# DCASE-REPO/DESED_task

Measured on AMD Instinct MI355X. Metric: 10s-clips/sec CRNN mean-teacher train @batch48, higher is better.
Workload: dtype f32 (fp32 storage and accumulation; the dense contractions of the wide layers run as split-bf16 MFMA, 3 bf16 products per fp32 product, fp32-level accuracy; everything else exact f32)

## Files before the change

### desed_task_amd/csrc/sed_glu.hip

```cpp
#include "sed_common.h"

#ifndef GLU_ABL
#define GLU_ABL 0
#endif

template <int C, int PT, int PF>
struct GluGeom {
    static constexpr int WIN = PT * PF;
    static constexpr int CP = C + 1;
    static constexpr int NT = C >= 32 ? C / 32 : 1;
};

template <int PT, int PF>
__device__ __forceinline__ bool row_pixel(int m, int o0, int NWC, int fsh, int& o, int& t, int& f) {
    constexpr int WIN = PT * PF;
    const int q = m % WIN;
    o = o0 + m / WIN;
    const int to = o >> fsh, fo = o & ((1 << fsh) - 1);
    t = to * PT + q / PF;
    f = fo * PF + q % PF;
    return o < NWC;
}

template <int C, int PT, int PF>
// ... 1711 lines not shown
                const int m = 16 * rb + 4 * g + r;
                const uint32_t e_idx = (uint32_t)(row0 + m) * (uint32_t)C + (uint32_t)n;
                const float xn = fmaf(xq[r], gn, bn);
                const float sg = (GLU_ABL & 2) ? xn : sed_fast_sigmoid(xn);
                const float lin = acc[rb][r] + biasp;
                const float gq = ((GLU_ABL & 2) || sed_keep(e_idx, seed, thr24)) ? g8[2 * rb + (r >> 1)] : 0.f;
                const float dlin = gq * sg;
                const float e = gq * lin * sg * (1.0f - sg);
                bf16_split(dlin, hh[r], ll[r]);
                dh[rm_off(m, n)] = hh[r];
                dl[rm_off(m, n)] = ll[r];
                acc[rb][r] = e;
                a_dbg += dlin;
            }
            uint2 hv, lv;
            hv.x = (unsigned)hh[0] | ((unsigned)hh[1] << 16); hv.y = (unsigned)hh[2] | ((unsigned)hh[3] << 16);
            lv.x = (unsigned)ll[0] | ((unsigned)ll[1] << 16); lv.y = (unsigned)ll[2] | ((unsigned)ll[3] << 16);
            const int off = tr_off(n, 16 * rb + 4 * g);
            *(uint2*)(dth + off) = hv;
            *(uint2*)(dtl + off) = lv;
        }
        __syncthreads();
        if (!(GLU_ABL & 1)) gemm_rows(dh, b2h, b2l, acc);
        const bool full = row0 + ROWS <= R;
#pragma unroll
        for (int rb = 0; rb < RB; ++rb) {
            float xq[4];
            xhat4(rb, xq);
#pragma unroll
            for (int r = 0; r < 4; ++r) {
                const int m = 16 * rb + 4 * g + r;
                const float dxn = acc[rb][r];
                a_dgam = fmaf(dxn, xq[r], a_dgam);
                a_dbet += dxn;
                if (!(GLU_ABL & 8) && (full || row0 + m < R)) dz[(size_t)(row0 + m) * C + n] = dxn * gn;
            }
        }
        if (tile + (int)gridDim.x < ntiles) load_tile(tile + gridDim.x);
        if (!(GLU_ABL & 1)) {
            const int rowa = 16 * w + i16;
            s16x8 ah3, al3;
#pragma unroll
            for (int st = 0; st < 2 * KS3; ++st) {
                const int ks = st >> 1, c0 = 4 * (st & 1);
                if ((st & 1) == 0) {
                    const int offa = tr_off(rowa, 32 * ks + 8 * g);
                    ah3 = *(const s16x8*)(dth + offa);
                    al3 = *(const s16x8*)(dtl + offa);
                }
                s16x8 bh3[4], bl3[4];
#pragma unroll
                for (int q = 0; q < 4; ++q) {
                    const int offb = tr_off(16 * (c0 + q) + i16, 32 * ks + 8 * g);
                    bh3[q] = *(const s16x8*)(xth + offb);
                    bl3[q] = *(const s16x8*)(xtl + offb);
                }
#pragma unroll
                for (int q = 0; q < 4; ++q) P[c0 + q] = mfma16_bf16(al3, bh3[q], P[c0 + q]);
#pragma unroll
                for (int q = 0; q < 4; ++q) P[c0 + q] = mfma16_bf16(ah3, bl3[q], P[c0 + q]);
#pragma unroll
                for (int q = 0; q < 4; ++q) P[c0 + q] = mfma16_bf16(ah3, bh3[q], P[c0 + q]);
                sed_sched_fence();
            }
        }
    }
    float* mine = part + (size_t)blockIdx.x * (C * C + 3 * C);
#pragma unroll
    for (int cb = 0; cb < NB; ++cb)
#pragma unroll
        for (int r = 0; r < 4; ++r) mine[(16 * w + 4 * g + r) * C + 16 * cb + i16] = P[cb][r];
    a_dbg += __shfl_xor(a_dbg, 16); a_dgam += __shfl_xor(a_dgam, 16); a_dbet += __shfl_xor(a_dbet, 16);
    a_dbg += __shfl_xor(a_dbg, 32); a_dgam += __shfl_xor(a_dgam, 32); a_dbet += __shfl_xor(a_dbet, 32);
    if (g == 0) {
        float* dst = mine + C * C;
        dst[n] = a_dbg; dst[C + n] = a_dgam; dst[2 * C + n] = a_dbet;
    }
}
#define GBR_THREADS 1024
#define GBR_GROUPS (GBR_THREADS / 16)
__global__ __launch_bounds__(GBR_THREADS) void glu_bwd_reduce_kernel(const float* __restrict__ part, float* __restrict__ dWg,
                                                             float* __restrict__ dbg, float* __restrict__ dgamma,
                                                             float* __restrict__ dbeta, int nblk, int C, int KS, int WMS,
                                                             const float* __restrict__ gamma, const float* __restrict__ beta, int fix) {
    __shared__ float4 red[GBR_GROUPS][16];
    __shared__ float sdb[GBR_THREADS / 64];
    const int tid = threadIdx.x, col = tid & 15, grp = tid >> 4, e = blockIdx.x * 64 + 4 * col;
    const int CC = C * C, PART = KS * CC + WMS * 3 * C;
    const bool isw = e < CC;
    const int nsl = isw ? KS : WMS, sstride = isw ? CC : 3 * C;
    const size_t off = isw ? (size_t)e : (size_t)KS * CC + (e - CC);
    float4 acc = make_float4(0.f, 0.f, 0.f, 0.f);
    if (e < CC + 3 * C) {
        const int total = nblk * nsl;
#pragma unroll 4
        for (int i = grp; i < total; i += GBR_GROUPS) {
            const int b = i / nsl, k = i - b * nsl;
            const float4 v = *(const float4*)(part + (size_t)b * PART + off + (size_t)k * sstride);
            acc.x += v.x; acc.y += v.y; acc.z += v.z; acc.w += v.w;
        }
    }
    const bool need_dbn = fix && blockIdx.x * 64 < CC;
    float sacc = 0.f;
    if (need_dbn) {
        const int nrow = (blockIdx.x * 64) / C;
#pragma unroll 2
        for (int i = tid; i < nblk * WMS; i += GBR_THREADS) {
            const int b = i / WMS, k = i - b * WMS;
            sacc += part[(size_t)b * PART + (size_t)KS * CC + k * 3 * C + nrow];
        }
    }
    float4 gq = make_float4(0.f, 0.f, 0.f, 0.f), bq = gq;
    if (fix && isw && grp == 0) {
        const int c = e % C;
        gq = make_float4(gamma[c], gamma[c + 1], gamma[c + 2], gamma[c + 3]);
        bq = make_float4(beta[c], beta[c + 1], beta[c + 2], beta[c + 3]);
    }
    red[grp][col] = acc;
    if (need_dbn) {
        sacc = wave_sum(sacc);
        if ((tid & 63) == 0) sdb[tid >> 6] = sacc;
    }
    __syncthreads();
    float dbn = 0.f;
    if (need_dbn) {
#pragma unroll
        for (int w = 0; w < GBR_THREADS / 64; ++w) dbn += sdb[w];
    }
    if (grp == 0 && e < CC + 3 * C) {
#pragma unroll 8
        for (int g = 1; g < GBR_GROUPS; ++g) { const float4 v = red[g][col]; acc.x += v.x; acc.y += v.y; acc.z += v.z; acc.w += v.w; }
        if (fix && isw) {
            acc.x = fmaf(gq.x, acc.x, bq.x * dbn); acc.y = fmaf(gq.y, acc.y, bq.y * dbn);
            acc.z = fmaf(gq.z, acc.z, bq.z * dbn); acc.w = fmaf(gq.w, acc.w, bq.w * dbn);
        }
        float* dst;
        if (isw) dst = dWg + e;
        else {
            const int j2 = e - CC, which = j2 / C;
            dst = (which == 0 ? dbg : which == 1 ? dgamma : dbeta) + (j2 - which * C);
        }
        *(float4*)dst = acc;
    }
}
template <int C, bool SPLIT>
static int launch_glu_wide_bwd(const float* y, const float* stats, const float* gamma, const float* beta, const float* Wg,
                               const float* bg, const float* gout, float* dz, float* dWg, float* dbg, float* dgamma, float* dbeta,
                               float* scratch, int B, int T, int F, uint32_t seed, uint32_t thr24, float dscale, const unsigned* seed_dev, hipStream_t s) {
    constexpr int ROWS = 32 * (8 / (C / 32)), WMS = 8 / (C / 32), KS = (C / 32) * (C / 32) >= 8 ? 1 : 8 / ((C / 32) * (C / 32));
    if (!scratch) return SED_ERR_ARG;
    constexpr int SMEM = SPLIT ? 8 * (ROWS * (C + 8) + C * (ROWS + 8)) : (2 * ROWS + (C > 64 ? C : 0)) * (C + 1) * 4;
    const int ntiles = (B * T * F + ROWS - 1) / ROWS;
    const int cap = glu_grid_cap(256);
    int grid = ntiles < cap ? ntiles : cap;
    if (grid < 1) { sed_zero4(s, dWg, C * C, dbg, C, dgamma, C, dbeta, C); return SED_OK; }
    if (SPLIT && C == 128 && sed_tuning[SED_TUNE_GLU_BWD128_SPLIT] != 1) {
        constexpr int SMEM_C = 8 * 64 * 128 * 2;
        SED_MAX_SMEM(glu128_bwd_c_kernel, SMEM_C);
        SED_LAUNCH(glu128_bwd_c_kernel, dim3(grid), dim3(512), SMEM_C, s, y, stats, gamma, beta, Wg, bg, gout, dz, scratch, B, T, F,
                   seed, thr24, dscale, seed_dev);
        SED_LAUNCH(glu_bwd_reduce_kernel, dim3((C * C + 3 * C + 63) / 64), dim3(GBR_THREADS), 0, s, scratch, dWg, dbg, dgamma, dbeta, grid, C, 1, 1,
                   gamma, beta, 1);
        return sed_check_launch();
    }
    if (SPLIT) {
        SED_MAX_SMEM((glu_wide_bwd_b_kernel<C>), SMEM);
        SED_LAUNCH((glu_wide_bwd_b_kernel<C>), dim3(grid), dim3(512), SMEM, s, y, stats, gamma, beta, Wg, bg, gout, dz, scratch, B, T, F,
                   seed, thr24, dscale, seed_dev);
    } else {
        SED_MAX_SMEM((glu_wide_bwd_kernel<C>), SMEM);
        SED_LAUNCH((glu_wide_bwd_kernel<C>), dim3(grid), dim3(512), SMEM, s, y, stats, gamma, beta, Wg, bg, gout, dz, scratch, B, T, F,
                   seed, thr24, dscale, seed_dev);
    }
    SED_LAUNCH(glu_bwd_reduce_kernel, dim3((C * C + 3 * C + 63) / 64), dim3(GBR_THREADS), 0, s, scratch, dWg, dbg, dgamma, dbeta, grid, C, KS, WMS,
               gamma, beta, SPLIT ? 1 : 0);
    return sed_check_launch();
}

SED_API long long sed_glu_bwd_scratch_floats(int B, int T, int F, int C, int PT, int PF) {
    (void)B; (void)T; (void)F;
    if (PT == 1 && PF == 2 && (C == 64 || C == 128)) {
        const int nt3 = (C / 32) * (C / 32), ks = nt3 >= 8 ? 1 : 8 / nt3, wms = 8 / (C / 32);
        return 256LL * (ks * C * C + wms * 3 * C);
    }
    if (PT == 2 && PF == 2 && (C == 16 || C == 32)) return 1024LL * (C * C + 3 * C);
    return 0;
}

SED_API int sed_glu_bwd(const float* y, const float* stats, const float* gamma, const float* beta, const float* Wg,
                           const float* bg, const float* gout, float* dz, float* dWg, float* dbg, float* dgamma, float* dbeta,
                           float* scratch, int B, int T, int F, int C, int PT, int PF, unsigned seed, unsigned thr24, float dscale,
                           const unsigned* seed_dev, int split_bf16, void* stream) {
    hipStream_t s = (hipStream_t)stream;
    if (F % PF != 0) return SED_ERR_UNSUPPORTED;
    if (PT == 1 && PF == 2) {
        if (C == 128 && split_bf16 && sed_tuning[SED_TUNE_GLU_BWD128_SPLIT] != 3)
            return launch_glu_wide_bwd<128, true>(y, stats, gamma, beta, Wg, bg, gout, dz, dWg, dbg, dgamma, dbeta, scratch, B, T, F, seed, thr24, dscale, seed_dev, s);
        if (C == 64 && split_bf16) return launch_glu_wide_bwd<64, true>(y, stats, gamma, beta, Wg, bg, gout, dz, dWg, dbg, dgamma, dbeta, scratch, B, T, F, seed, thr24, dscale, seed_dev, s);
        if (C == 128) return launch_glu_wide_bwd<128, false>(y, stats, gamma, beta, Wg, bg, gout, dz, dWg, dbg, dgamma, dbeta, scratch, B, T, F, seed, thr24, dscale, seed_dev, s);
        if (C == 64) return launch_glu_wide_bwd<64, false>(y, stats, gamma, beta, Wg, bg, gout, dz, dWg, dbg, dgamma, dbeta, scratch, B, T, F, seed, thr24, dscale, seed_dev, s);
    }
    const bool lds_free32 = C == 32 && PT == 2 && PF == 2 && F % 16 == 0 && T >= 2;
    if (T % PT != 0 && !lds_free32) {
        const int tail = T % PT, rowf4 = F * C / 4;
        const long long n4 = (long long)B * tail * rowf4;
        int grid = (int)((n4 + 255) / 256);
        if (grid > 2048) grid = 2048;
        SED_LAUNCH(glu_zero_tail_kernel, dim3(grid), dim3(256), 0, s, dz, n4, T, T - tail, tail * rowf4, (long long)T * rowf4);
    }
    if ((C == 16 && PT == 2 && PF == 2 && F % 8 == 0) || (C == 32 && PT == 2 && PF == 2 && F % 16 == 0)) {
        const int nrows = B * (T / 2);
        int grid = (nrows + 3) / 4;
        const int cap = C == 32 ? glu_grid_cap(512) : 1024;
        if (grid > cap) grid = cap;
        if (grid < 1) { sed_zero4(s, dWg, C * C, dbg, C, dgamma, C, dbeta, C); return SED_OK; }
        if (!scratch) return SED_ERR_ARG;
        if (C == 16)
            SED_LAUNCH(glu16_bwd_kernel, dim3(grid), dim3(256), 0, s, y, stats, gamma, beta, Wg, bg, gout, dz, scratch, B, T, F, seed, thr24,
                       dscale, seed_dev);
        else
            SED_LAUNCH(glu32_bwd_kernel, dim3(grid), dim3(256), 0, s, y, stats, gamma, beta, Wg, bg, gout, dz, scratch, B, T, F, seed, thr24,
                       dscale, seed_dev);
        SED_LAUNCH(glu_bwd_reduce_kernel, dim3((C * C + 3 * C + 63) / 64), dim3(GBR_THREADS), 0, s, scratch, dWg, dbg, dgamma, dbeta, grid, C, 1, 1,
                   gamma, beta, 0);
        return sed_check_launch();
    }
    sed_zero4(s, dWg, C * C, dbg, C, dgamma, C, dbeta, C);
#define GLU_CASE(c, pt, pf)                                                                                              \
    if (C == c && PT == pt && PF == pf)                                                                                  \
        return launch_glu_bwd<c, pt, pf>(y, stats, gamma, beta, Wg, bg, gout, dz, dWg, dbg, dgamma, dbeta, B, T, F, seed, thr24, \
                                         dscale, seed_dev, s);
    GLU_CASE(16, 2, 2) GLU_CASE(32, 2, 2)
#undef GLU_CASE
    return SED_ERR_UNSUPPORTED;
}

template <int C>
__global__ __launch_bounds__(256) void bn_bwd_apply_kernel(const float* __restrict__ y, float* __restrict__ dz,
                                                           const float* __restrict__ stats, const float* __restrict__ gamma,
                                                           const float* __restrict__ dgamma, const float* __restrict__ dbeta,
                                                           float* __restrict__ dbias, size_t npix, float inv_count, int training) {
    constexpr int V = C / 4, RPI = 256 / V;
    const int tid = threadIdx.x, v = tid % V, r0 = tid / V;
    float mean[4], istd[4], m1[4], m2[4];
#pragma unroll
    for (int i = 0; i < 4; ++i) {
        const int c = 4 * v + i;
        mean[i] = stats[c];
        istd[i] = stats[C + c];
        m1[i] = training ? gamma[c] * dbeta[c] * inv_count : 0.f;
        m2[i] = training ? gamma[c] * dgamma[c] * inv_count : 0.f;
    }
    if (blockIdx.x == 0 && tid < C) dbias[tid] = training ? 0.f : stats[C + tid] * gamma[tid] * dbeta[tid];
    for (size_t p = (size_t)blockIdx.x * RPI + r0; p < npix; p += (size_t)gridDim.x * RPI) {
        const float4 yv = *(const float4*)(y + p * C + 4 * v);
        float4 g = *(const float4*)(dz + p * C + 4 * v);
        g.x = istd[0] * (g.x - m1[0] - (yv.x - mean[0]) * istd[0] * m2[0]);
        g.y = istd[1] * (g.y - m1[1] - (yv.y - mean[1]) * istd[1] * m2[1]);
        g.z = istd[2] * (g.z - m1[2] - (yv.z - mean[2]) * istd[2] * m2[2]);
        g.w = istd[3] * (g.w - m1[3] - (yv.w - mean[3]) * istd[3] * m2[3]);
        *(float4*)(dz + p * C + 4 * v) = g;
    }
}
SED_API int sed_bn_bwd_apply(const float* y, float* dz, const float* stats, const float* gamma, const float* dgamma,
                                const float* dbeta, float* dbias, long long npix, int C, int training, void* stream) {
    hipStream_t s = (hipStream_t)stream;
    if (npix <= 0) return SED_OK;
    const float inv = 1.0f / (float)npix;
    int grid = (int)((npix * (C / 4) + 255) / 256);
    if (grid > 4096) grid = 4096;
#define BN_CASE(c) \
    if (C == c) { SED_LAUNCH((bn_bwd_apply_kernel<c>), dim3(grid), dim3(256), 0, s, y, dz, stats, gamma, dgamma, dbeta, dbias, (size_t)npix, inv, training); return sed_check_launch(); }
    BN_CASE(16) BN_CASE(32) BN_CASE(64) BN_CASE(128)
#undef BN_CASE
    return SED_ERR_UNSUPPORTED;
}
```

### desed_task_amd/ops.py

```python
import os

import torch

from . import _lib
from . import graph as _graph

BN_EPS = 1e-3
BN_MOMENTUM = 0.99
BLOCK0_FUSED = os.environ.get("SED_BLOCK0_FUSED", "1") != "0"
BN_BWD_FOLD = os.environ.get("SED_BN_BWD_FOLD", "1") != "0"


GRU_DW_ATOMIC = False

GRU_DW_SIDE = False
GRU_WIDE = os.environ.get("SED_GRU_WIDE", "0") == "1"
GRU_DX_SPLITK = True
GRU_DW_SIDE_ALLOWED = True
CNN_DW_SIDE = os.environ.get("SED_CNN_DW_SIDE", "1") != "0"
CNN_DW_SIDE_NOW = True
_side = {}



PROBE = None


def probe(tag):
    if PROBE is not None:
        PROBE(tag)


def side_stream(device):
    if device.type != "cuda":
        return None
    key = (device.type, device.index)
    if key not in _side:
        _side[key] = torch.cuda.Stream(device=device)
    return _side[key]


def join_side_stream(device):
    s = _side.get((device.type, device.index))
    if _deferred:
        flush_deferred(s)
    if s is not None:
        torch.cuda.current_stream(device).wait_stream(s)


AFTER_FORWARD = None
PARK_LOSS_SUMS = True


def run_after_forward(parked, side):
    for launch, keep in parked:
        if side is None:
            launch(_lib.stream_ptr(keep[0]))
            continue
        for t in keep:
            t.record_stream(side)
        with torch.cuda.stream(side):
            launch(side.cuda_stream)


_deferred = []
DEFER_OFF_CHAIN = True


SIDE_ON_CPU = False


def defer_off_chain(device, launch, keep):
    if GRU_DW_SIDE and DEFER_OFF_CHAIN and (device.type == "cuda" or SIDE_ON_CPU):
        fork = None
        if device.type == "cuda":
            fork = torch.cuda.Event()
            fork.record(torch.cuda.current_stream(device))
        _deferred.append((launch, keep, fork))
    else:
        launch(_lib.stream_ptr(keep[0]))


def flush_deferred(side):
    todo, _deferred[:] = list(_deferred), []
    for launch, keep, fork in todo:
        if side is not None:
            side.wait_event(fork)
            for t in keep:
                t.record_stream(side)
            with torch.cuda.stream(side):
                launch(side.cuda_stream)
        else:
            launch(_lib.stream_ptr(keep[0]))


PRECISIONS = ("f32", "bf16x3", "bf16")
_SUFFIX = {"f32": "", "bf16x3": "_bf16x3", "bf16": "_bf16x1"}


def gemm_suffix(cfg):
    prec = (cfg or {}).get("gemm_precision") or os.environ.get("SED_GEMM_PRECISION", "bf16x3")
    if prec not in PRECISIONS:
# ... 180 lines not shown
                nblk = lib.value("sed_conv_fwd_blocks", B, T, F, CIN, COUT)
                partial = torch.empty(nblk * 2 * COUT, device=dev, dtype=torch.float32)
                lib.call("sed_conv0_fwd", x.data_ptr(), conv_w.data_ptr(), _p(conv_b), _p(bounds), None, partial.data_ptr(),
                         B, T, F, COUT, st)
            lib.call("sed_bn_finalize", _p(partial), nblk, COUT, float(B * T * F), bn_w.data_ptr(), bn_b.data_ptr(),
                     running_mean.data_ptr(), running_var.data_ptr(), BN_MOMENTUM, BN_EPS, stats.data_ptr(), int(training),
                     int(training and cfg.get("update_running", True)), st)
            out = torch.empty(B, T // PT, F // PF, COUT, device=dev, dtype=torch.float32)
            glu_w = glu_w.contiguous()
            lib.call("sed_block0_fwd", x.data_ptr(), conv_w.data_ptr(), _p(conv_b), _p(bounds), stats.data_ptr(), glu_w.data_ptr(),
                     glu_b.data_ptr(), out.data_ptr(), B, T, F, int(seed), thr24, dscale, _graph.seed_dev(seed), st)
            ctx.save_for_backward(x, stats, conv_w, bn_w, bn_b, glu_w, glu_b, conv_b)
            ctx.meta = (first, B, T, F, CIN, COUT, PT, PF, training, seed, thr24, dscale, bounds)
            ctx.cfg = cfg
            ctx.fused0 = True
            return out
        ctx.fused0 = False
        y = torch.empty(B, T, F, COUT, device=dev, dtype=torch.float32)
        prec = cfg.get("conv_precision", "f32")
        bf16x3 = (not first) and _mfma_bf16(prec) and cfg.get("packed") is not None
        sfx = _SUFFIX[prec] if bf16x3 else ""
        nblk = lib.value("sed_conv_fwd_blocks_bf16" if bf16x3 else "sed_conv_fwd_blocks", B, T, F, CIN, COUT)
        partial = torch.empty(nblk * 2 * COUT, device=dev, dtype=torch.float32) if training else None
        conv_w = conv_w.contiguous()
        if first:
            lib.call("sed_conv0_fwd", x.data_ptr(), conv_w.data_ptr(), _p(conv_b), _p(bounds), y.data_ptr(), _p(partial),
                     B, T, F, COUT, st)
        else:
            packed = cfg.get("packed")
            if packed is not None:
                wf = packed[0]
            else:
                wf = torch.empty(9 * CIN * COUT, device=dev, dtype=torch.float32)
                lib.call("sed_conv_pack_weights", conv_w.data_ptr(), wf.data_ptr(), None, COUT, CIN, st)
            lib.call("sed_conv3x3" + sfx, x.data_ptr(), wf.data_ptr(), _p(conv_b), y.data_ptr(), _p(partial), B, T, F, CIN, COUT, st)
        stats = torch.empty(4 * COUT, device=dev, dtype=torch.float32)
        lib.call("sed_bn_finalize", _p(partial), nblk, COUT, float(B * T * F), bn_w.data_ptr(), bn_b.data_ptr(),
                 running_mean.data_ptr(), running_var.data_ptr(), BN_MOMENTUM, BN_EPS, stats.data_ptr(), int(training),
                 int(training and cfg.get("update_running", True)), st)
        out = torch.empty(B, T // PT, F // PF, COUT, device=dev, dtype=torch.float32)
        glu_w = glu_w.contiguous()
        lib.call("sed_glu_fwd", y.data_ptr(), stats.data_ptr(), glu_w.data_ptr(), glu_b.data_ptr(), out.data_ptr(), B, T, F, COUT,
                 PT, PF, int(seed), thr24, dscale, _graph.seed_dev(seed), int(_mfma_bf16(prec)), st)
        ctx.save_for_backward(x, y, stats, conv_w, bn_w, bn_b, glu_w, glu_b, conv_b)
        ctx.meta = (first, B, T, F, CIN, COUT, PT, PF, training, seed, thr24, dscale, bounds)
        ctx.cfg = cfg
        return out

    @staticmethod
    def backward(ctx, gout):
        lib = _lib.get()
        probe("convblock_bwd")
        if ctx.fused0:
            x, stats, conv_w, bn_w, bn_b, glu_w, glu_b, conv_b = ctx.saved_tensors
            first, B, T, F, CIN, COUT, PT, PF, training, seed, thr24, dscale, bounds = ctx.meta
            cfg = ctx.cfg
            gout = gout.contiguous()
            st = _lib.stream_ptr(x)
            d_w, d_bias = _grad_buf(cfg, conv_w), _grad_buf(cfg, conv_b)
            d_gamma, d_beta = _grad_buf(cfg, bn_w), _grad_buf(cfg, bn_b)
            d_glu_w, d_glu_b = _grad_buf(cfg, glu_w), _grad_buf(cfg, glu_b)
            scratch = torch.empty(int(lib.value("sed_block0_bwd_scratch_floats", B, T, F)), device=x.device, dtype=torch.float32)
            lib.call("sed_block0_bwd", x.data_ptr(), conv_w.data_ptr(), _p(conv_b), _p(bounds), stats.data_ptr(), bn_w.data_ptr(),
                     bn_b.data_ptr(), glu_w.data_ptr(), glu_b.data_ptr(), gout.data_ptr(), d_w.data_ptr(), d_bias.data_ptr(),
                     d_gamma.data_ptr(), d_beta.data_ptr(), d_glu_w.data_ptr(), d_glu_b.data_ptr(), scratch.data_ptr(), B, T, F,
                     int(seed), thr24, dscale, _graph.seed_dev(seed), st)
            if _deferred:
                flush_deferred(side_stream(x.device) if GRU_DW_SIDE else None)
            return None, d_w, d_bias, d_gamma, d_beta, d_glu_w, d_glu_b, None, None, None
        x, y, stats, conv_w, bn_w, bn_b, glu_w, glu_b, conv_b = ctx.saved_tensors
        first, B, T, F, CIN, COUT, PT, PF, training, seed, thr24, dscale, bounds = ctx.meta
        gout = gout.contiguous()
        dev = y.device
        st = _lib.stream_ptr(y)
        f32 = dict(device=dev, dtype=torch.float32)
        dz = torch.empty_like(y)
        cfg = ctx.cfg
        d_glu_w = _grad_buf(cfg, glu_w)
        d_glu_b = _grad_buf(cfg, glu_b)
        d_gamma = _grad_buf(cfg, bn_w)
        d_beta = _grad_buf(cfg, bn_b)
        nscr = int(lib.value("sed_glu_bwd_scratch_floats", B, T, F, COUT, PT, PF))
        gscratch = torch.empty(nscr, **f32) if nscr else None
        lib.call("sed_glu_bwd", y.data_ptr(), stats.data_ptr(), bn_w.data_ptr(), bn_b.data_ptr(), glu_w.data_ptr(), glu_b.data_ptr(),
                 gout.data_ptr(), dz.data_ptr(), d_glu_w.data_ptr(), d_glu_b.data_ptr(), d_gamma.data_ptr(), d_beta.data_ptr(),
                 _p(gscratch), B, T, F, COUT, PT, PF, int(seed), thr24, dscale, _graph.seed_dev(seed),
                 int(_mfma_bf16(cfg.get("conv_precision", "f32"))), st)
        if _deferred:
            flush_deferred(side_stream(dev) if GRU_DW_SIDE else None)
        d_bias = _grad_buf(cfg, conv_b)
        d_w = _grad_buf(cfg, conv_w)
        dx = None
        if first and training:
            lib.call("sed_conv0_wgrad", x.data_ptr(), _p(bounds), dz.data_ptr(), y.data_ptr(), stats.data_ptr(), bn_w.data_ptr(),
                     d_gamma.data_ptr(), d_beta.data_ptr(), d_w.data_ptr(), d_bias.data_ptr(), B, T, F, COUT, 1, 1, st)
            return dx, d_w, d_bias, d_gamma, d_beta, d_glu_w, d_glu_b, None, None, None
        packed = cfg.get("packed")
        prec = cfg.get("conv_precision", "f32")
        sfx = _SUFFIX[prec]
        if (BN_BWD_FOLD and training and not first and ctx.needs_input_grad[0] and _mfma_bf16(prec)
                and packed is not None and packed[1] is not None):
            dy = torch.empty_like(dz)
            dx = torch.empty_like(x)
            lib.call("sed_conv3x3%s_bnbwd" % sfx, dz.data_ptr(), y.data_ptr(), stats.data_ptr(), bn_w.data_ptr(), d_gamma.data_ptr(),
                     d_beta.data_ptr(), packed[1].data_ptr(), dx.data_ptr(), dy.data_ptr(), d_bias.data_ptr(), B, T, F, COUT, CIN, st)
            scratch = torch.empty(int(lib.value("sed_conv_wgrad_scratch_floats", B, T, F, CIN, COUT)), **f32)
            d_w_ptr = d_w.data_ptr()

            def wgrad(stream_ptr):
                lib.call("sed_conv_wgrad" + sfx, x.data_ptr(), dy.data_ptr(), scratch.data_ptr(), d_w_ptr, B, T, F, CIN, COUT, stream_ptr)
            if CNN_DW_SIDE and CNN_DW_SIDE_NOW and _arena_views(cfg, d_w):
                defer_off_chain(dev, wgrad, (x, dy, scratch))
            else:
                wgrad(st)
            return dx, d_w, d_bias, d_gamma, d_beta, d_glu_w, d_glu_b, None, None, None
        lib.call("sed_bn_bwd_apply", y.data_ptr(), dz.data_ptr(), stats.data_ptr(), bn_w.data_ptr(), d_gamma.data_ptr(),
                 d_beta.data_ptr(), d_bias.data_ptr(), B * T * F, COUT, int(training), st)
        dy = dz
        if first:
            lib.call("sed_conv0_wgrad", x.data_ptr(), _p(bounds), dy.data_ptr(), None, None, None, None, None, d_w.data_ptr(), None,
                     B, T, F, COUT, 0, int(training), st)
        else:
            scratch = torch.empty(int(lib.value("sed_conv_wgrad_scratch_floats", B, T, F, CIN, COUT)), **f32)
            lib.call("sed_conv_wgrad" + sfx, x.data_ptr(), dy.data_ptr(), scratch.data_ptr(), d_w.data_ptr(), B, T, F, CIN, COUT, st)
            if ctx.needs_input_grad[0]:
                packed = cfg.get("packed")
                bf16x3 = False
                if packed is not None and packed[1] is not None:
                    wd = packed[1]
                    bf16x3 = _mfma_bf16(prec)
                else:
                    wd = torch.empty(9 * CIN * COUT, **f32)
                    wf = torch.empty(9 * CIN * COUT, **f32)
                    lib.call("sed_conv_pack_weights", conv_w.data_ptr(), wf.data_ptr(), wd.data_ptr(), COUT, CIN, st)
                dx = torch.empty_like(x)
                lib.call("sed_conv3x3" + (sfx if bf16x3 else ""), dy.data_ptr(), wd.data_ptr(), None, dx.data_ptr(), None, B, T, F, COUT, CIN, st)
        return dx, d_w, d_bias, d_gamma, d_beta, d_glu_w, d_glu_b, None, None, None


def _gemm(lib, A, Bm, bias, C, M, N, K, lda, ldb, ldc, ta, tb, split_k, accumulate, st):
    lib.call("sed_gemm", A, Bm, bias, C, M, N, K, lda, ldb, ldc, ta, tb, split_k, accumulate, st)


class BiGRULayerFn(torch.autograd.Function):

    @staticmethod
    def forward(ctx, x, w_ih_f, w_hh_f, b_ih_f, b_hh_f, w_ih_r, w_hh_r, b_ih_r, b_hh_r, cfg=None):
        lib = _lib.get()
        x = x.contiguous()
        _lib.check_tensor(x, "gru input")
        B, T, I = x.shape
        H = w_hh_f.shape[1]
        st = _lib.stream_ptr(x)
        f32 = dict(device=x.device, dtype=torch.float32)
        gi = torch.empty(B, T, 2, 3 * H, **f32)
        w_ih = [w_ih_f.contiguous(), w_ih_r.contiguous()]
        w_hh = [w_hh_f.contiguous(), w_hh_r.contiguous()]
        lib.call(gemm_entry(cfg), x.data_ptr(), x.data_ptr(), w_ih[0].data_ptr(), w_ih[1].data_ptr(), b_ih_f.data_ptr(),
                 b_ih_r.data_ptr(), gi.data_ptr(), gi.data_ptr() + 3 * H * 4, B * T, 3 * H, I, I, I, 6 * H, 0, 1, 1, 0, st)
        out = torch.empty(B, T, 2 * H, **f32)
        need = any(ctx.needs_input_grad)
        saved = torch.empty(B, T, 2, 4, H, **f32) if need else None
        lib.call("sed_gru_fwd", gi.data_ptr(), w_hh[0].data_ptr(), w_hh[1].data_ptr(), b_hh_f.data_ptr(), b_hh_r.data_ptr(),
                 out.data_ptr(), _p(saved), B, T, H, st)
        if need:
            ctx.save_for_backward(x, out, saved, w_ih[0], w_ih[1], w_hh[0], w_hh[1], b_ih_f, b_hh_f, b_ih_r, b_hh_r)
        ctx.dims = (B, T, I, H)
        ctx.cfg = cfg
        return out

    @staticmethod
    def backward(ctx, dout):
# ... 302 lines not shown
```

### include/sed_hip.h

```cpp
#ifndef SED_HIP_H
#define SED_HIP_H

#ifdef __cplusplus
extern "C" {
#endif

int sed_mel_fwd(const float* audio, float* out, int B, int N, int T, int n_fft, int hop, int n_mels,
                const float* window, const float* tw1024, const float* tw2048, const int* fb_start,
                const int* fb_len, const float* fb_w, int fb_stride, int apply_log, void* stream);

int sed_mel_taps(const int* fb_start, const int* fb_len, const float* fb_w, int fb_stride, int n_mels, float* taps, void* stream);
int sed_mel_fwd_wave(const float* audio, float* out, int B, int N, int T, int n_fft, int hop, int n_mels,
                     const float* window, const float* tw1024, const float* tw2048, const int* fb_start,
                     const int* fb_len, const float* fb_w, int fb_stride, const float* taps, int apply_log, void* stream);

int sed_logscale_fwd(const float* x, float* logbuf, float* out, float* partial, float* minmax, int B, int L,
                     int apply_log, float eps, void* stream);

int sed_take_log(const float* x, float* y, long long n, void* stream);


int sed_mixup(float* data, float* tmp, const int* perm, float c, float one_minus_c, int n, int L, int mode,
              const float* c_dev, void* stream);

int sed_mixup_multi(const long long* jobs, int njobs, void* stream);

int sed_specaug(const float* x, float* y, const int* bounds, int B, int T, int Fq, void* stream);

int sed_specaug_bounds(const float* u_f, const float* u_t, int* bounds, int B, int n, int f_param, int n_freq, int t_param,
                       int n_time, void* stream);

int sed_specaug_bounds_seeded(int* bounds, int B, int n, int f_param, int n_freq, int t_param, int n_time, unsigned seed,
                              const unsigned* seed_dev, void* stream);

int sed_weak_labels(const float* labels, float* out, int n, int NC, int T, void* stream);


int sed_conv_pack_weights(const float* W, float* Wf, float* Wd, int COUT, int CIN, void* stream);

int sed_conv_pack_multi(int n, const void* const* W, void* const* Wf, void* const* Wd, const int* cout, const int* cin,
                        void* stream);

int sed_conv_fwd_blocks(int B, int T, int F, int CIN, int COUT);

int sed_conv3x3(const float* x, const float* Wp, const float* bias, float* y, float* partial, int B, int T, int F,
                int CIN, int COUT, void* stream);

int sed_conv_pack_multi_bf16(int n, const void* const* W, void* const* Wf, void* const* Wd, const int* cout,
                             const int* cin, void* stream);
int sed_conv3x3_bf16x3(const float* x, const void* Wp, const float* bias, float* y, float* partial, int B, int T, int F,
                       int CIN, int COUT, void* stream);
int sed_cnn_prologue_bf16(int n, const void* const* W, void* const* Wf, void* const* Wd, const int* cout, const int* cin,
                          int* bounds, int B, int nb, int f_param, int n_freq, int t_param, int n_time, unsigned seed,
                          const unsigned* seed_dev, const float* copy_src, float* copy_dst, long long copy_n, void* stream);

int sed_conv3x3_bf16x3_bnbwd(const float* dz, const float* ybn, const float* stats, const float* gamma, const float* dgamma,
                             const float* dbeta, const void* Wd, float* dx, float* dy_out, float* dbias, int B, int T, int F,
                             int CIN, int COUT, void* stream);
int sed_conv_fwd_blocks_bf16(int B, int T, int F, int CIN, int COUT);

int sed_conv_pack_multi_bf16x1(int n, const void* const* W, void* const* Wf, void* const* Wd, const int* cout,
                               const int* cin, void* stream);
int sed_conv3x3_bf16x1(const float* x, const void* Wp, const float* bias, float* y, float* partial, int B, int T, int F,
                       int CIN, int COUT, void* stream);
int sed_cnn_prologue_bf16x1(int n, const void* const* W, void* const* Wf, void* const* Wd, const int* cout, const int* cin,
                            int* bounds, int B, int nb, int f_param, int n_freq, int t_param, int n_time, unsigned seed,
                            const unsigned* seed_dev, const float* copy_src, float* copy_dst, long long copy_n, void* stream);
int sed_conv3x3_bf16x1_bnbwd(const float* dz, const float* ybn, const float* stats, const float* gamma, const float* dgamma,
                             const float* dbeta, const void* Wd, float* dx, float* dy_out, float* dbias, int B, int T, int F,
                             int CIN, int COUT, void* stream);

int sed_conv0_fwd(const float* x, const float* W, const float* bias, const int* bounds, float* y, float* partial,
                  int B, int T, int F, int COUT, void* stream);

int sed_block0_fwd(const float* x, const float* W, const float* bias, const int* bounds, const float* stats, const float* Wg,
                   const float* bg, float* out, int B, int T, int F, unsigned seed, unsigned thr24, float dscale,
                   const unsigned* seed_dev, void* stream);
long long sed_block0_bwd_scratch_floats(int B, int T, int F);
int sed_block0_bwd(const float* x, const float* W, const float* bias, const int* bounds, const float* stats, const float* gamma,
                   const float* beta, const float* Wg, const float* bg, const float* gout, float* dW, float* dbias, float* dgamma,
                   float* dbeta, float* dWg, float* dbg, float* scratch, int B, int T, int F, unsigned seed, unsigned thr24,
                   float dscale, const unsigned* seed_dev, void* stream);

int sed_bn_finalize(const float* partial, int nblocks, int C, float count, const float* gamma, const float* beta,
                    float* running_mean, float* running_var, float momentum, float eps, float* stats, int training,
                    int update_running, void* stream);

int sed_glu_fwd(const float* y, const float* stats, const float* Wg, const float* bg, float* out, int B, int T, int F,
                int C, int PT, int PF, unsigned seed, unsigned thr24, float dscale, const unsigned* seed_dev, int split_bf16,
                void* stream);

long long sed_glu_bwd_scratch_floats(int B, int T, int F, int C, int PT, int PF);

int sed_glu_bwd(const float* y, const float* stats, const float* gamma, const float* beta, const float* Wg,
                const float* bg, const float* gout, float* dz, float* dWg, float* dbg, float* dgamma, float* dbeta,
                float* scratch, int B, int T, int F, int C, int PT, int PF, unsigned seed, unsigned thr24, float dscale,
                const unsigned* seed_dev, int split_bf16, void* stream);

int sed_bn_bwd_apply(const float* y, float* dz, const float* stats, const float* gamma, const float* dgamma,
                     const float* dbeta, float* dbias, long long npix, int C, int training, void* stream);

long long sed_conv_wgrad_scratch_floats(int B, int T, int F, int CIN, int COUT);

int sed_conv_wgrad(const float* x, const float* dy, float* dWp, float* dW, int B, int T, int F, int CIN, int COUT,
                   void* stream);

int sed_conv_wgrad_bf16x3(const float* x, const float* dy, float* dWp, float* dW, int B, int T, int F, int CIN, int COUT,
                          void* stream);
int sed_conv_wgrad_bf16x1(const float* x, const float* dy, float* dWp, float* dW, int B, int T, int F, int CIN, int COUT,
                          void* stream);

int sed_conv0_wgrad(const float* x, const int* bounds, const float* dyz, const float* y, const float* stats,
                    const float* gamma, const float* dgamma, const float* dbeta, float* dW, float* dbias, int B, int T,
                    int F, int COUT, int fuse_bn, int training, void* stream);


int sed_gemm(const float* A, const float* Bm, const float* bias, float* Cm, int M, int N, int K, int lda, int ldb,
             int ldc, int transA, int transB, int split_k, int accumulate, void* stream);

int sed_gemm_pair(const float* A0, const float* A1, const float* B0, const float* B1, const float* bias0,
                  const float* bias1, float* C0, float* C1, int M, int N, int K, int lda, int ldb, int ldc, int transA,
                  int transB, int split_k, int accumulate, void* stream);

int sed_gemm_bf16x3(const float* A, const float* Bm, const float* bias, float* Cm, int M, int N, int K, int lda, int ldb,
                    int ldc, int transA, int transB, int split_k, int accumulate, void* stream);
int sed_gemm_kcat(const float* A, const float* B0, const float* B1, float* Cm, int M, int N, int K, int ksplit, int lda,
                  int ldb, int ldc, void* stream);
int sed_gemm_kcat_bf16x3(const float* A, const float* B0, const float* B1, float* Cm, int M, int N, int K, int ksplit, int lda,
                         int ldb, int ldc, void* stream);
int sed_gemm_kcat_splitk_bf16x3(const float* A, const float* B0, const float* B1, float* Cm, int M, int N, int K, int ksplit,
                                int lda, int ldb, int ldc, int split_k, float* scratch, void* stream);
int sed_gemm_pair_bf16x3(const float* A0, const float* A1, const float* B0, const float* B1, const float* bias0,
                         const float* bias1, float* C0, float* C1, int M, int N, int K, int lda, int ldb, int ldc,
                         int transA, int transB, int split_k, int accumulate, void* stream);
long long sed_gemm_splitk_scratch_floats(int M, int N, int K, int split_k);
int sed_gemm_pair_splitk_bf16x3(const float* A0, const float* A1, const float* B0, const float* B1, float* C0, float* C1,
                                int M, int N, int K, int lda, int ldb, int ldc, int transA, int transB, int split_k,
                                float* scratch, void* stream);
int sed_gemm_splitk_bf16x3(const float* A, const float* Bm, float* Cm, int M, int N, int K, int lda, int ldb, int ldc,
                           int transA, int transB, int split_k, float* scratch, void* stream);

int sed_gemm_bf16x1(const float* A, const float* Bm, const float* bias, float* Cm, int M, int N, int K, int lda, int ldb,
                    int ldc, int transA, int transB, int split_k, int accumulate, void* stream);
int sed_gemm_pair_bf16x1(const float* A0, const float* A1, const float* B0, const float* B1, const float* bias0,
                         const float* bias1, float* C0, float* C1, int M, int N, int K, int lda, int ldb, int ldc,
                         int transA, int transB, int split_k, int accumulate, void* stream);
int sed_gemm_kcat_bf16x1(const float* A, const float* B0, const float* B1, float* Cm, int M, int N, int K, int ksplit, int lda,
                         int ldb, int ldc, void* stream);
int sed_gemm_kcat_splitk_bf16x1(const float* A, const float* B0, const float* B1, float* Cm, int M, int N, int K, int ksplit,
                                int lda, int ldb, int ldc, int split_k, float* scratch, void* stream);
int sed_gemm_pair_splitk_bf16x1(const float* A0, const float* A1, const float* B0, const float* B1, float* C0, float* C1,
                                int M, int N, int K, int lda, int ldb, int ldc, int transA, int transB, int split_k,
                                float* scratch, void* stream);
int sed_gemm_splitk_bf16x1(const float* A, const float* Bm, float* Cm, int M, int N, int K, int lda, int ldb, int ldc,
                           int transA, int transB, int split_k, float* scratch, void* stream);

int sed_colsum(const float* X, float* out, float* out1, int nsplit, int M, int N, int ld, void* stream);

int sed_gru_fwd(const float* gi, const float* whh0, const float* whh1, const float* bhh0, const float* bhh1,
                float* out, float* saved, int B, int T, int H, void* stream);

int sed_gru_bwd(const float* dout, const float* out, const float* saved, const float* whh0, const float* whh1,
                float* dgi, float* dgh, float* hprev, float* dbi0, float* dbi1, float* dbh0, float* dbh1, int B, int T, int H,
                float* scratch, void* stream);
int sed_gru_bias_reduce(const float* scratch, float* dbi0, float* dbi1, float* dbh0, float* dbh1, int B, int H, void* stream);


int sed_head_fwd(const float* x, const float* W1, const float* b1, const float* W2, const float* b2, float* strong,
                 float* psoft, float* weak, float* den, int B, int T, int D, int NC, unsigned seed, unsigned thr24,
                 float dscale, const unsigned* seed_dev, const unsigned char* classes_valid, const unsigned char* pad_mask,
                 void* stream);

int sed_head_bwd(const float* x, const float* W1, const float* W2, const float* strong, const float* psoft,
                 const float* weak, const float* den, const float* d_strong, const float* d_weak, float* dx, float* dW1,
                 float* dW2, float* db1, float* db2, int B, int T, int D, int NC, unsigned seed, unsigned thr24,
                 float dscale, const unsigned* seed_dev, const unsigned char* classes_valid, const unsigned char* pad_mask,
                 float* scratch, void* stream);
long long sed_head_bwd_scratch_floats(int B, int T, int D, int NC);
int sed_head_bwd_reduce(const float* scratch, float* dW1, float* dW2, float* db1, float* db2, int B, int T, int D, int NC,
                        void* stream);
// ... 93 lines not shown
```

Baseline: 16610.

## Split GLU backward reduce so weight-gradient half runs off the critical chain

Splits the GLU backward reduction kernel into a chain half (bias, gamma, beta grads needed downstream) and a weight half (dWg) by adding a block offset. The weight half is deferred to a side stream through the existing off-chain mechanism. The aim is to shorten the serial backward critical path by overlapping the dWg reduction with later layers. In exchange it adds an extra kernel launch and keeps the scratch buffer alive longer, and the reduction now has to be correctly ordered across streams.

```diff
diff --git a/desed_task_amd/csrc/sed_glu.hip b/desed_task_amd/csrc/sed_glu.hip
--- a/desed_task_amd/csrc/sed_glu.hip
+++ b/desed_task_amd/csrc/sed_glu.hip
@@ -1817,10 +1817,12 @@
 __global__ __launch_bounds__(GBR_THREADS) void glu_bwd_reduce_kernel(const float* __restrict__ part, float* __restrict__ dWg,
                                                              float* __restrict__ dbg, float* __restrict__ dgamma,
                                                              float* __restrict__ dbeta, int nblk, int C, int KS, int WMS,
-                                                             const float* __restrict__ gamma, const float* __restrict__ beta, int fix) {
+                                                             const float* __restrict__ gamma, const float* __restrict__ beta, int fix,
+                                                             int blk0) {
     __shared__ float4 red[GBR_GROUPS][16];
     __shared__ float sdb[GBR_THREADS / 64];
-    const int tid = threadIdx.x, col = tid & 15, grp = tid >> 4, e = blockIdx.x * 64 + 4 * col;
+    const int blk = blk0 + blockIdx.x;
+    const int tid = threadIdx.x, col = tid & 15, grp = tid >> 4, e = blk * 64 + 4 * col;
     const int CC = C * C, PART = KS * CC + WMS * 3 * C;
     const bool isw = e < CC;
     const int nsl = isw ? KS : WMS, sstride = isw ? CC : 3 * C;
@@ -1835,10 +1837,10 @@
             acc.x += v.x; acc.y += v.y; acc.z += v.z; acc.w += v.w;
         }
     }
-    const bool need_dbn = fix && blockIdx.x * 64 < CC;
+    const bool need_dbn = fix && blk * 64 < CC;
     float sacc = 0.f;
     if (need_dbn) {
-        const int nrow = (blockIdx.x * 64) / C;
+        const int nrow = (blk * 64) / C;
 #pragma unroll 2
         for (int i = tid; i < nblk * WMS; i += GBR_THREADS) {
             const int b = i / WMS, k = i - b * WMS;
@@ -1878,96 +1880,149 @@
         *(float4*)dst = acc;
     }
 }
+enum { GLU_BWD_NONE = 0, GLU_BWD_ATOMIC = 1, GLU_BWD_WIDE = 2, GLU_BWD_NARROW = 3 };
+struct GluBwdPlan {
+    int kind;
+    int grid;
+    int KS, WMS, fix;
+    bool split, ckernel;
+};
+static GluBwdPlan glu_bwd_plan(int B, int T, int F, int C, int PT, int PF, int split_bf16) {
+    GluBwdPlan p = {GLU_BWD_NONE, 0, 1, 1, 0, false, false};
+    if (PF <= 0 || F % PF != 0) return p;
+    if (PT == 1 && PF == 2 && (C == 64 || C == 128)) {
+        const int nt = C / 32, rows = 32 * (8 / nt);
+        p.kind = GLU_BWD_WIDE;
+        p.split = split_bf16 && !(C == 128 && sed_tuning[SED_TUNE_GLU_BWD128_SPLIT] == 3);
+        p.ckernel = p.split && C == 128 && sed_tuning[SED_TUNE_GLU_BWD128_SPLIT] != 1;
+        p.WMS = p.ckernel ? 1 : 8 / nt;
+        p.KS = p.ckernel || nt * nt >= 8 ? 1 : 8 / (nt * nt);
+        p.fix = p.split ? 1 : 0;
+        const int ntiles = (B * T * F + rows - 1) / rows;
+        const int cap = glu_grid_cap(256);
+        p.grid = ntiles < cap ? ntiles : cap;
+        return p;
+    }
+    if ((C == 16 && PT == 2 && PF == 2 && F % 8 == 0) || (C == 32 && PT == 2 && PF == 2 && F % 16 == 0)) {
+        const int nrows = B * (T / 2);
+        const int cap = C == 32 ? glu_grid_cap(512) : 1024;
+        p.kind = GLU_BWD_NARROW;
+        p.grid = (nrows + 3) / 4;
+        if (p.grid > cap) p.grid = cap;
+        return p;
+    }
+    if ((C == 16 || C == 32) && PT == 2 && PF == 2) p.kind = GLU_BWD_ATOMIC;
+    return p;
+}
+
+enum { GLU_HALF_CHAIN = 1, GLU_HALF_WEIGHT = 2 };
+static void launch_glu_reduce(hipStream_t s, const float* scratch, float* dWg, float* dbg, float* dgamma, float* dbeta,
+                              const GluBwdPlan& p, int C, const float* gamma, const float* beta, int halves) {
+    const int wblk = C * C / 64, nb = (C * C + 3 * C + 63) / 64;
+    const int first = (halves & GLU_HALF_WEIGHT) ? 0 : wblk, last = (halves & GLU_HALF_CHAIN) ? nb : wblk;
+    SED_LAUNCH(glu_bwd_reduce_kernel, dim3(last - first), dim3(GBR_THREADS), 0, s, scratch, dWg, dbg, dgamma, dbeta, p.grid, C, p.KS, p.WMS,
+               gamma, beta, p.fix, first);
+}
+
 template <int C, bool SPLIT>
-static int launch_glu_wide_bwd(const float* y, const float* stats, const float* gamma, const float* beta, const float* Wg,
-                               const float* bg, const float* gout, float* dz, float* dWg, float* dbg, float* dgamma, float* dbeta,
-                               float* scratch, int B, int T, int F, uint32_t seed, uint32_t thr24, float dscale, const unsigned* seed_dev, hipStream_t s) {
-    constexpr int ROWS = 32 * (8 / (C / 32)), WMS = 8 / (C / 32), KS = (C / 32) * (C / 32) >= 8 ? 1 : 8 / ((C / 32) * (C / 32));
-    if (!scratch) return SED_ERR_ARG;
+static void launch_glu_wide_bwd(const GluBwdPlan& p, const float* y, const float* stats, const float* gamma, const float* beta,
+                                const float* Wg, const float* bg, const float* gout, float* dz, float* scratch, int B, int T, int F,
+                                uint32_t seed, uint32_t thr24, float dscale, const unsigned* seed_dev, hipStream_t s) {
+    constexpr int ROWS = 32 * (8 / (C / 32));
     constexpr int SMEM = SPLIT ? 8 * (ROWS * (C + 8) + C * (ROWS + 8)) : (2 * ROWS + (C > 64 ? C : 0)) * (C + 1) * 4;
-    const int ntiles = (B * T * F + ROWS - 1) / ROWS;
-    const int cap = glu_grid_cap(256);
-    int grid = ntiles < cap ? ntiles : cap;
-    if (grid < 1) { sed_zero4(s, dWg, C * C, dbg, C, dgamma, C, dbeta, C); return SED_OK; }
-    if (SPLIT && C == 128 && sed_tuning[SED_TUNE_GLU_BWD128_SPLIT] != 1) {
+    if (SPLIT && C == 128 && p.ckernel) {
         constexpr int SMEM_C = 8 * 64 * 128 * 2;
         SED_MAX_SMEM(glu128_bwd_c_kernel, SMEM_C);
-        SED_LAUNCH(glu128_bwd_c_kernel, dim3(grid), dim3(512), SMEM_C, s, y, stats, gamma, beta, Wg, bg, gout, dz, scratch, B, T, F,
+        SED_LAUNCH(glu128_bwd_c_kernel, dim3(p.grid), dim3(512), SMEM_C, s, y, stats, gamma, beta, Wg, bg, gout, dz, scratch, B, T, F,
                    seed, thr24, dscale, seed_dev);
-        SED_LAUNCH(glu_bwd_reduce_kernel, dim3((C * C + 3 * C + 63) / 64), dim3(GBR_THREADS), 0, s, scratch, dWg, dbg, dgamma, dbeta, grid, C, 1, 1,
-                   gamma, beta, 1);
-        return sed_check_launch();
-    }
-    if (SPLIT) {
+    } else if (SPLIT) {
         SED_MAX_SMEM((glu_wide_bwd_b_kernel<C>), SMEM);
-        SED_LAUNCH((glu_wide_bwd_b_kernel<C>), dim3(grid), dim3(512), SMEM, s, y, stats, gamma, beta, Wg, bg, gout, dz, scratch, B, T, F,
+        SED_LAUNCH((glu_wide_bwd_b_kernel<C>), dim3(p.grid), dim3(512), SMEM, s, y, stats, gamma, beta, Wg, bg, gout, dz, scratch, B, T, F,
                    seed, thr24, dscale, seed_dev);
     } else {
         SED_MAX_SMEM((glu_wide_bwd_kernel<C>), SMEM);
-        SED_LAUNCH((glu_wide_bwd_kernel<C>), dim3(grid), dim3(512), SMEM, s, y, stats, gamma, beta, Wg, bg, gout, dz, scratch, B, T, F,
+        SED_LAUNCH((glu_wide_bwd_kernel<C>), dim3(p.grid), dim3(512), SMEM, s, y, stats, gamma, beta, Wg, bg, gout, dz, scratch, B, T, F,
                    seed, thr24, dscale, seed_dev);
     }
-    SED_LAUNCH(glu_bwd_reduce_kernel, dim3((C * C + 3 * C + 63) / 64), dim3(GBR_THREADS), 0, s, scratch, dWg, dbg, dgamma, dbeta, grid, C, KS, WMS,
-               gamma, beta, SPLIT ? 1 : 0);
-    return sed_check_launch();
 }
 
 SED_API long long sed_glu_bwd_scratch_floats(int B, int T, int F, int C, int PT, int PF) {
-    (void)B; (void)T; (void)F;
-    if (PT == 1 && PF == 2 && (C == 64 || C == 128)) {
-        const int nt3 = (C / 32) * (C / 32), ks = nt3 >= 8 ? 1 : 8 / nt3, wms = 8 / (C / 32);
-        return 256LL * (ks * C * C + wms * 3 * C);
-    }
-    if (PT == 2 && PF == 2 && (C == 16 || C == 32)) return 1024LL * (C * C + 3 * C);
+    const GluBwdPlan p = glu_bwd_plan(B, T, F, C, PT, PF, 0);
+    if (p.kind == GLU_BWD_WIDE) return 256LL * (p.KS * C * C + p.WMS * 3 * C);
+    if (p.kind == GLU_BWD_NARROW) return 1024LL * (C * C + 3 * C);
     return 0;
 }
 
-SED_API int sed_glu_bwd(const float* y, const float* stats, const float* gamma, const float* beta, const float* Wg,
-                           const float* bg, const float* gout, float* dz, float* dWg, float* dbg, float* dgamma, float* dbeta,
-                           float* scratch, int B, int T, int F, int C, int PT, int PF, unsigned seed, unsigned thr24, float dscale,
-                           const unsigned* seed_dev, int split_bf16, void* stream) {
-    hipStream_t s = (hipStream_t)stream;
-    if (F % PF != 0) return SED_ERR_UNSUPPORTED;
-    if (PT == 1 && PF == 2) {
-        if (C == 128 && split_bf16 && sed_tuning[SED_TUNE_GLU_BWD128_SPLIT] != 3)
-            return launch_glu_wide_bwd<128, true>(y, stats, gamma, beta, Wg, bg, gout, dz, dWg, dbg, dgamma, dbeta, scratch, B, T, F, seed, thr24, dscale, seed_dev, s);
-        if (C == 64 && split_bf16) return launch_glu_wide_bwd<64, true>(y, stats, gamma, beta, Wg, bg, gout, dz, dWg, dbg, dgamma, dbeta, scratch, B, T, F, seed, thr24, dscale, seed_dev, s);
-        if (C == 128) return launch_glu_wide_bwd<128, false>(y, stats, gamma, beta, Wg, bg, gout, dz, dWg, dbg, dgamma, dbeta, scratch, B, T, F, seed, thr24, dscale, seed_dev, s);
-        if (C == 64) return launch_glu_wide_bwd<64, false>(y, stats, gamma, beta, Wg, bg, gout, dz, dWg, dbg, dgamma, dbeta, scratch, B, T, F, seed, thr24, dscale, seed_dev, s);
-    }
+static int glu_bwd_run(int halves, bool partials_only, const float* y, const float* stats, const float* gamma, const float* beta,
+                       const float* Wg, const float* bg, const float* gout, float* dz, float* dWg, float* dbg, float* dgamma,
+                       float* dbeta, float* scratch, int B, int T, int F, int C, int PT, int PF, unsigned seed, unsigned thr24,
+                       float dscale, const unsigned* seed_dev, int split_bf16, hipStream_t s) {
+    const GluBwdPlan p = glu_bwd_plan(B, T, F, C, PT, PF, split_bf16);
+    if (p.kind == GLU_BWD_NONE || (partials_only && p.kind == GLU_BWD_ATOMIC)) return SED_ERR_UNSUPPORTED;
+    if ((p.kind == GLU_BWD_WIDE || partials_only) && !scratch) return SED_ERR_ARG;
+    const bool chain = (halves & GLU_HALF_CHAIN) != 0, weight = (halves & GLU_HALF_WEIGHT) != 0;
     const bool lds_free32 = C == 32 && PT == 2 && PF == 2 && F % 16 == 0 && T >= 2;
-    if (T % PT != 0 && !lds_free32) {
+    if (chain && T % PT != 0 && !lds_free32) {
         const int tail = T % PT, rowf4 = F * C / 4;
         const long long n4 = (long long)B * tail * rowf4;
         int grid = (int)((n4 + 255) / 256);
         if (grid > 2048) grid = 2048;
         SED_LAUNCH(glu_zero_tail_kernel, dim3(grid), dim3(256), 0, s, dz, n4, T, T - tail, tail * rowf4, (long long)T * rowf4);
     }
-    if ((C == 16 && PT == 2 && PF == 2 && F % 8 == 0) || (C == 32 && PT == 2 && PF == 2 && F % 16 == 0)) {
-        const int nrows = B * (T / 2);
-        int grid = (nrows + 3) / 4;
-        const int cap = C == 32 ? glu_grid_cap(512) : 1024;
-        if (grid > cap) grid = cap;
-        if (grid < 1) { sed_zero4(s, dWg, C * C, dbg, C, dgamma, C, dbeta, C); return SED_OK; }
-        if (!scratch) return SED_ERR_ARG;
-        if (C == 16)
-            SED_LAUNCH(glu16_bwd_kernel, dim3(grid), dim3(256), 0, s, y, stats, gamma, beta, Wg, bg, gout, dz, scratch, B, T, F, seed, thr24,
-                       dscale, seed_dev);
-        else
-            SED_LAUNCH(glu32_bwd_kernel, dim3(grid), dim3(256), 0, s, y, stats, gamma, beta, Wg, bg, gout, dz, scratch, B, T, F, seed, thr24,
-                       dscale, seed_dev);
-        SED_LAUNCH(glu_bwd_reduce_kernel, dim3((C * C + 3 * C + 63) / 64), dim3(GBR_THREADS), 0, s, scratch, dWg, dbg, dgamma, dbeta, grid, C, 1, 1,
-                   gamma, beta, 0);
-        return sed_check_launch();
-    }
-    sed_zero4(s, dWg, C * C, dbg, C, dgamma, C, dbeta, C);
+    if (p.kind == GLU_BWD_ATOMIC) {
+        sed_zero4(s, dWg, C * C, dbg, C, dgamma, C, dbeta, C);
 #define GLU_CASE(c, pt, pf)                                                                                              \
     if (C == c && PT == pt && PF == pf)                                                                                  \
         return launch_glu_bwd<c, pt, pf>(y, stats, gamma, beta, Wg, bg, gout, dz, dWg, dbg, dgamma, dbeta, B, T, F, seed, thr24, \
                                          dscale, seed_dev, s);
-    GLU_CASE(16, 2, 2) GLU_CASE(32, 2, 2)
+        GLU_CASE(16, 2, 2) GLU_CASE(32, 2, 2)
 #undef GLU_CASE
-    return SED_ERR_UNSUPPORTED;
+        return SED_ERR_UNSUPPORTED;
+    }
+    if (p.grid < 1) {
+        sed_zero4(s, weight ? dWg : nullptr, weight ? C * C : 0, dbg, chain ? C : 0, dgamma, chain ? C : 0, dbeta, chain ? C : 0);
+        return SED_OK;
+    }
+    if (!scratch) return SED_ERR_ARG;
+    if (chain) {
+        if (p.kind == GLU_BWD_WIDE) {
+            if (C == 128 && p.split) launch_glu_wide_bwd<128, true>(p, y, stats, gamma, beta, Wg, bg, gout, dz, scratch, B, T, F, seed, thr24, dscale, seed_dev, s);
+            else if (C == 128) launch_glu_wide_bwd<128, false>(p, y, stats, gamma, beta, Wg, bg, gout, dz, scratch, B, T, F, seed, thr24, dscale, seed_dev, s);
+            else if (p.split) launch_glu_wide_bwd<64, true>(p, y, stats, gamma, beta, Wg, bg, gout, dz, scratch, B, T, F, seed, thr24, dscale, seed_dev, s);
+            else launch_glu_wide_bwd<64, false>(p, y, stats, gamma, beta, Wg, bg, gout, dz, scratch, B, T, F, seed, thr24, dscale, seed_dev, s);
+        } else if (C == 16) {
+            SED_LAUNCH(glu16_bwd_kernel, dim3(p.grid), dim3(256), 0, s, y, stats, gamma, beta, Wg, bg, gout, dz, scratch, B, T, F, seed, thr24,
+                       dscale, seed_dev);
+        } else {
+            SED_LAUNCH(glu32_bwd_kernel, dim3(p.grid), dim3(256), 0, s, y, stats, gamma, beta, Wg, bg, gout, dz, scratch, B, T, F, seed, thr24,
+                       dscale, seed_dev);
+        }
+    }
+    launch_glu_reduce(s, scratch, weight ? dWg : nullptr, chain ? dbg : nullptr, chain ? dgamma : nullptr, chain ? dbeta : nullptr, p, C,
+                      gamma, beta, halves);
+    return sed_check_launch();
+}
+
+SED_API int sed_glu_bwd(const float* y, const float* stats, const float* gamma, const float* beta, const float* Wg,
+                           const float* bg, const float* gout, float* dz, float* dWg, float* dbg, float* dgamma, float* dbeta,
+                           float* scratch, int B, int T, int F, int C, int PT, int PF, unsigned seed, unsigned thr24, float dscale,
+                           const unsigned* seed_dev, int split_bf16, void* stream) {
+    return glu_bwd_run(GLU_HALF_CHAIN | GLU_HALF_WEIGHT, false, y, stats, gamma, beta, Wg, bg, gout, dz, dWg, dbg, dgamma, dbeta, scratch,
+                       B, T, F, C, PT, PF, seed, thr24, dscale, seed_dev, split_bf16, (hipStream_t)stream);
+}
+
+SED_API int sed_glu_bwd_chain(const float* y, const float* stats, const float* gamma, const float* beta, const float* Wg,
+                                 const float* bg, const float* gout, float* dz, float* dbg, float* dgamma, float* dbeta, float* scratch,
+                                 int B, int T, int F, int C, int PT, int PF, unsigned seed, unsigned thr24, float dscale,
+                                 const unsigned* seed_dev, int split_bf16, void* stream) {
+    return glu_bwd_run(GLU_HALF_CHAIN, true, y, stats, gamma, beta, Wg, bg, gout, dz, nullptr, dbg, dgamma, dbeta, scratch, B, T, F, C, PT, PF,
+                       seed, thr24, dscale, seed_dev, split_bf16, (hipStream_t)stream);
+}
+
+SED_API int sed_glu_bwd_weights(const float* scratch, float* dWg, const float* gamma, const float* beta, int B, int T, int F, int C,
+                                   int PT, int PF, int split_bf16, void* stream) {
+    return glu_bwd_run(GLU_HALF_WEIGHT, true, nullptr, nullptr, gamma, beta, nullptr, nullptr, nullptr, nullptr, dWg, nullptr, nullptr,
+                       nullptr, const_cast<float*>(scratch), B, T, F, C, PT, PF, 0u, 0u, 1.f, nullptr, split_bf16, (hipStream_t)stream);
 }
 
 template <int C>
diff --git a/desed_task_amd/ops.py b/desed_task_amd/ops.py
--- a/desed_task_amd/ops.py
+++ b/desed_task_amd/ops.py
@@ -18,6 +18,7 @@
 GRU_DX_SPLITK = True
 GRU_DW_SIDE_ALLOWED = True
 CNN_DW_SIDE = os.environ.get("SED_CNN_DW_SIDE", "1") != "0"
+GLU_DW_OFF_CHAIN = os.environ.get("SED_GLU_DW_OFF_CHAIN", "1") != "0"
 CNN_DW_SIDE_NOW = True
 _side = {}
 
@@ -364,12 +365,25 @@
         d_beta = _grad_buf(cfg, bn_b)
         nscr = int(lib.value("sed_glu_bwd_scratch_floats", B, T, F, COUT, PT, PF))
         gscratch = torch.empty(nscr, **f32) if nscr else None
-        lib.call("sed_glu_bwd", y.data_ptr(), stats.data_ptr(), bn_w.data_ptr(), bn_b.data_ptr(), glu_w.data_ptr(), glu_b.data_ptr(),
-                 gout.data_ptr(), dz.data_ptr(), d_glu_w.data_ptr(), d_glu_b.data_ptr(), d_gamma.data_ptr(), d_beta.data_ptr(),
-                 _p(gscratch), B, T, F, COUT, PT, PF, int(seed), thr24, dscale, _graph.seed_dev(seed),
-                 int(_mfma_bf16(cfg.get("conv_precision", "f32"))), st)
+        split = int(_mfma_bf16(cfg.get("conv_precision", "f32")))
+        dw_off_chain = GLU_DW_OFF_CHAIN and nscr > 0 and CNN_DW_SIDE and CNN_DW_SIDE_NOW and _arena_views(cfg, d_glu_w)
+        if dw_off_chain:
+            lib.call("sed_glu_bwd_chain", y.data_ptr(), stats.data_ptr(), bn_w.data_ptr(), bn_b.data_ptr(), glu_w.data_ptr(), glu_b.data_ptr(),
+                     gout.data_ptr(), dz.data_ptr(), d_glu_b.data_ptr(), d_gamma.data_ptr(), d_beta.data_ptr(), gscratch.data_ptr(),
+                     B, T, F, COUT, PT, PF, int(seed), thr24, dscale, _graph.seed_dev(seed), split, st)
+        else:
+            lib.call("sed_glu_bwd", y.data_ptr(), stats.data_ptr(), bn_w.data_ptr(), bn_b.data_ptr(), glu_w.data_ptr(), glu_b.data_ptr(),
+                     gout.data_ptr(), dz.data_ptr(), d_glu_w.data_ptr(), d_glu_b.data_ptr(), d_gamma.data_ptr(), d_beta.data_ptr(),
+                     _p(gscratch), B, T, F, COUT, PT, PF, int(seed), thr24, dscale, _graph.seed_dev(seed), split, st)
         if _deferred:
             flush_deferred(side_stream(dev) if GRU_DW_SIDE else None)
+        if dw_off_chain:
+            d_glu_w_ptr = d_glu_w.data_ptr()
+
+            def glu_dw(stream_ptr):
+                lib.call("sed_glu_bwd_weights", gscratch.data_ptr(), d_glu_w_ptr, bn_w.data_ptr(), bn_b.data_ptr(), B, T, F, COUT, PT, PF,
+                         split, stream_ptr)
+            defer_off_chain(dev, glu_dw, (gscratch,))
         d_bias = _grad_buf(cfg, conv_b)
         d_w = _grad_buf(cfg, conv_w)
         dx = None
diff --git a/include/sed_hip.h b/include/sed_hip.h
--- a/include/sed_hip.h
+++ b/include/sed_hip.h
@@ -96,6 +96,13 @@
                 const float* bg, const float* gout, float* dz, float* dWg, float* dbg, float* dgamma, float* dbeta,
                 float* scratch, int B, int T, int F, int C, int PT, int PF, unsigned seed, unsigned thr24, float dscale,
                 const unsigned* seed_dev, int split_bf16, void* stream);
+
+int sed_glu_bwd_chain(const float* y, const float* stats, const float* gamma, const float* beta, const float* Wg,
+                      const float* bg, const float* gout, float* dz, float* dbg, float* dgamma, float* dbeta, float* scratch,
+                      int B, int T, int F, int C, int PT, int PF, unsigned seed, unsigned thr24, float dscale,
+                      const unsigned* seed_dev, int split_bf16, void* stream);
+int sed_glu_bwd_weights(const float* scratch, float* dWg, const float* gamma, const float* beta, int B, int T, int F, int C,
+                        int PT, int PF, int split_bf16, void* stream);
 
 int sed_bn_bwd_apply(const float* y, float* dz, const float* stats, const float* gamma, const float* dgamma,
                      const float* dbeta, float* dbias, long long npix, int C, int training, void* stream);
```

After: 16690 (median of 6 runs). Within noise of the previous version (+0.4%).
